# mfkiwl/coxgraph

Measured on AMD Instinct MI355X. Metric: 640x480 depth frames/sec fused (TSDF, 5 cm voxels) per node; submap registrations/sec reported alongside, higher is better.
Workload: dtype f32; 1 GPU; configs[1]: 1 client per GPU, 640x480 synthetic depth stream, 5 cm voxels, merged integrator semantics (the reference's configured method is fast; bit-exact vs CPU oracle), points resident in HBM; points_per_frame=307200, method=merged, clients=1

## Files before the change

coxgraph_amd/csrc/cox_integrator.hip:

```cpp
#include <hip/hip_runtime.h>

#include <algorithm>
#include <chrono>
#include <cmath>
#include <cstring>
#include <limits>
#include <new>
#include <string>
#include <vector>

#include "../../include/coxgraph_hip_history.h"
#include "../../include/coxgraph_hip_selftest.h"
#include "cox_host.hpp"
#include "cox_plan.hpp"
#include "cox_sort.hpp"
#include "cox_threads.hpp"

using namespace cox;
using cox_plan::IntegratorPlan;
using cox_plan::LayerUpdate;

#include "cox_frame.hpp"
#include "cox_raygen.hpp"
#include "cox_walk.hpp"
#include "cox_pieces.hpp"
#include "cox_fast.hpp"
#include "cox_apply_records.hpp"
#include "cox_apply_tile.hpp"
#include "cox_frontend.hpp"

static_assert(cox_plan::kAxisCapSmall == kAxisCapSmall && cox_plan::kTileShift == kTileShift && cox_plan::kBigChunk == kBigChunk &&
                  cox_plan::kBigChunkMin == kBigChunkMin && cox_plan::kFastMaxRounds == kFastMaxRounds && cox_plan::kFastShortMax == kFastShortMax &&
                  cox_plan::kFastRelaxGroups == kFastRelaxGroups && cox_plan::kCopyGroups == kCopyGroups,
              "cox_plan.hpp decides with the kernels' own constants");

constexpr int kStatRing = 8;
constexpr int kFrameSets = 6;
constexpr int kStageSets = 3;
constexpr int kInputSets = kFrameSets;
using cox_plan::kNumStages;

struct FrameSet {
  FrameParams* d_params = nullptr;
  Counters* cnt = nullptr;
  RayArrays rays{};
  u64* fh_keys = nullptr;
  u32* fh_first = nullptr;
  hipEvent_t done = nullptr;
  hipEvent_t params_copied = nullptr;
  hipEvent_t hand[kNumStages - 1] = {};
  bool used = false;
};
struct BundleSet {
  u32 *pslot = nullptr, *skey[2] = {nullptr, nullptr}, *sval[2] = {nullptr, nullptr}, *bstart = nullptr;
  u32 *hrank = nullptr, *head = nullptr;
  SortInfo* sort_info = nullptr;
  hipEvent_t done = nullptr;
  bool used = false;
};
struct RecordSet {
  u32 *rec_key[2] = {nullptr, nullptr}, *rec_ray[2] = {nullptr, nullptr};
  u32 *piece_front = nullptr, *piece_back = nullptr, *piece_wsum = nullptr;
  uint8_t* lin8 = nullptr;
  u32 *pkey[2] = {nullptr, nullptr}, *pstart[2] = {nullptr, nullptr}, *prl[2] = {nullptr, nullptr};
  u64* pbkey = nullptr;
  u32 *plen = nullptr, *pdest = nullptr;
  u32* touched_slots = nullptr;
  u64* ft_keys = nullptr;
  u32* ft_ord = nullptr;
  int4* ord_info = nullptr;
  u32 *blk_beg = nullptr, *blk_end = nullptr;
  u32 *big_of_tile = nullptr, *big_acc = nullptr;
  u32* blk_list = nullptr;
  uint2* big_chunks = nullptr;
  u32 big_chunk_cap = 0;
  SortInfo* sort_info = nullptr;
  hipEvent_t done = nullptr;
// ... 390 lines not shown
static int points_sort_passes(const cox_integrator* I) { return (ceil_log2(next_pow2(static_cast<u64>(I->pcap) + 1)) + 1 + 10) / 11; }

static int stage_hash(const StageCtx& c, hipStream_t s) {
  cox_integrator* I = c.I;
  FrameSet& F = *c.F;
  BundleSet& B = *c.B;
  const bool by_value = (I->method == COX_METHOD_MERGED) && !I->graphs_on;
  if (!by_value) {
    COX_HIP(hipMemcpyAsync(F.d_params, &I->h_params[c.slot], sizeof(FrameParams), hipMemcpyHostToDevice, s));
    if (c.n_dev) hipLaunchKernelGGL(k_params_count, dim3(1), dim3(1), 0, s, F.d_params, c.n_dev);
  }
  COX_HIP(hipMemsetAsync(F.cnt, 0, sizeof(Counters), s));
  if (I->method == COX_METHOD_MERGED) {
    const u32 n = I->pcap;
    {
      TimedRegion t(I, COX_KC_BUNDLE_HASH, s);
      const bool self_clean = !I->cfg.enable_anti_grazing;
      if (!self_clean) COX_HIP(hipMemsetAsync(F.fh_keys, 0xFF, sizeof(u64) * I->fh_cap + sizeof(u32) * I->fh_cap, s));
      hipLaunchKernelGGL(k_bundle_insert, grid_for(n), dim3(256), 0, s, F.d_params, I->h_params[c.slot], by_value ? 1 : 0, c.n_dev, F.fh_keys, F.fh_first,
                         I->fh_cap - 1, B.pslot, F.cnt);
    }
  }
  return COX_OK;
}
static int stage_point_sort(const StageCtx& c, hipStream_t s) {
  cox_integrator* I = c.I;
  FrameSet& F = *c.F;
  BundleSet& B = *c.B;
  if (I->method == COX_METHOD_MERGED) {
    const u32 n = I->pcap;
    const SortWorkspace& ws = (I->st_alt && (c.slot & 1)) ? I->sort_pts_alt : I->sort_pts;
    const bool counted = static_cast<u64>(n) <= static_cast<u64>(kRsMaxTiles) * kRsTile;
    {
      TimedRegion t(I, COX_KC_BUNDLE_HASH, s);
      hipLaunchKernelGGL(k_bundle_keys, grid_for(n, kHeadTile), dim3(kKeysThreads), 0, s, F.d_params, F.fh_keys, F.fh_first, B.pslot, B.skey[0], B.sval[0], B.hrank, B.head,
                         B.sort_info, counted ? ws.counts : nullptr, ws.totals);
    }
    const bool self_clean = !I->cfg.enable_anti_grazing;
    const BundleBounds bounds{F.d_params, B.head, B.hrank, B.pslot, B.bstart, F.cnt, self_clean ? F.fh_keys : nullptr, F.fh_first, I->fh_cap - 1};
    TimedRegion t(I, COX_KC_POINT_SORT, s);
    (void)radix_sort_pairs<11, BundleBounds>(B.skey[0], B.sval[0], B.skey[1], B.sval[1], &F.d_params->n_points, n, n, 0, true, points_sort_passes(I), ws, B.sort_info,
                                             s, nullptr, nullptr, counted, bounds);
  }
  return COX_OK;
}
static FrameBlocks frame_blocks(const cox_integrator* I, const RecordSet& S) { return FrameBlocks{S.ft_keys, S.ft_ord, S.touched_slots, I->layer->ht_cap - 1}; }
static void record_walk(const StageCtx& c, hipStream_t s) {
  cox_integrator* I = c.I;
  const IntegratorPlan& P = I->plan;
  FrameSet& F = *c.F;
  RecordSet& S = *c.S;
  const u32 fh_mask = I->fh_cap - 1;
  const FrameBlocks FB = frame_blocks(I, S);
  if (P.small_axis_cap)
    hipLaunchKernelGGL(k_touch_wave<kAxisCapSmall>, dim3(P.grid_touch), dim3(256), 0, s, F.d_params, F.rays, FB, S.rec_key[1], I->rcap, F.cnt, F.fh_keys, fh_mask);
  else
    hipLaunchKernelGGL(k_touch_wave<kAxisCapLarge>, dim3(2048), dim3(256), 0, s, F.d_params, F.rays, FB, S.rec_key[1], I->rcap, F.cnt, F.fh_keys, fh_mask);
  hipLaunchKernelGGL(k_emit_wave, dim3(P.grid_touch), dim3(256), 0, s, F.d_params, F.rays, FB, S.rec_key[1], S.rec_key[0], S.rec_ray[0], I->rcap, F.cnt, S.sort_info,
                     F.fh_keys, fh_mask, P.emit_flags());
}
static bool binds_in_apply(const cox_integrator* I) { return I->method == COX_METHOD_MERGED && I->plan.layer_update == LayerUpdate::RecordTiles; }
static void bind_blocks(const StageCtx& c, hipStream_t s) {
  cox_integrator* I = c.I;
  if (binds_in_apply(I)) return;
  hipLaunchKernelGGL(k_bind_blocks, dim3(16), dim3(256), 0, s, layer_view(I->layer), frame_blocks(I, *c.S), c.S->ord_info, c.F->cnt, I->layer->d_err);
}
static int stage_merge(const StageCtx& c, hipStream_t s) {
  cox_integrator* I = c.I;
  FrameSet& F = *c.F;
  BundleSet& B = *c.B;
  const u32 n = I->pcap;
  if (I->method == COX_METHOD_MERGED) {
    BundleView V{{B.skey[0], B.skey[1]}, {B.sval[0], B.sval[1]}, B.sort_info};
    {
      TimedRegion t(I, COX_KC_MERGE, s);
      hipLaunchKernelGGL(k_bundle_merge, dim3(I->plan.grid_merge), dim3(256), 0, s, F.d_params, V, B.bstart, F.rays, F.cnt,
                         I->plan.walks_pieces() ? (I->plan.small_axis_cap ? kAxisCapSmall : kAxisCapLarge) : 0u);
    }
    const bool odd = I->st_alt && (c.slot & 1);
    const ScanWorkspace& ws = odd ? I->scanws_a : I->scanws_b;
    if (!I->plan.walks_pieces()) {
      hipLaunchKernelGGL(k_scan_small, dim3(1), dim3(1024), 0, s, F.rays.nsteps, F.rays.rec_off, &F.cnt->n_ray_slots, I->pcap, &F.cnt->n_records);
    } else if (I->plan.small_axis_cap) {
      hipLaunchKernelGGL(k_scan_small2, dim3(1), dim3(1024), 0, s, F.rays.nsteps, F.rays.rec_off, &F.cnt->n_records, F.rays.pbound, F.rays.piece_off,
                         &F.cnt->n_piece_slots, &F.cnt->n_ray_slots, I->pcap);
    } else {
      exclusive_scan_u32(F.rays.nsteps, F.rays.rec_off, &F.cnt->n_ray_slots, I->pcap, I->pcap, &F.cnt->n_records, ws, s);
      exclusive_scan_u32(F.rays.pbound, F.rays.piece_off, &F.cnt->n_ray_slots, I->pcap, I->pcap, &F.cnt->n_piece_slots, ws, s);
    }
  } else {
    hipLaunchKernelGGL(k_rays_simple, grid_for(n), dim3(256), 0, s, F.d_params, F.rays, F.cnt);
  }
  return COX_OK;
}
static int stage_touch(const StageCtx& c, hipStream_t s) {
  cox_integrator* I = c.I;
  const IntegratorPlan& P = I->plan;
  FrameSet& F = *c.F;
  RecordSet& S = *c.S;
  const LayerView L = layer_view(I->layer);
  const u32 fh_mask = I->fh_cap - 1;
  if (P.walk_on_raygen) {
    bind_blocks(c, s);
    return COX_OK;
  }
  TimedRegion t_walk(I, COX_KC_TOUCH_EMIT, s);
  if (P.walks_pieces()) {
    const PieceArrays PA{S.pkey[0], S.pstart[0], S.prl[0], S.pbkey};
#define COX_LAUNCH_WALK(CAP, DEFER)                                                                                                                       \
  hipLaunchKernelGGL((k_touch_pieces<CAP, DEFER>), dim3(2048), dim3(256), 0, s, F.d_params, F.rays, L, S.touched_slots, S.lin8, PA, I->rcap, I->piece_cap, \
                     F.cnt, I->layer->d_err)
    if (P.expands_pieces()) {
      if (P.small_axis_cap)
        COX_LAUNCH_WALK(kAxisCapSmall, true);
      else
        COX_LAUNCH_WALK(kAxisCapLarge, true);
      hipLaunchKernelGGL(k_piece_touch, dim3(2048), dim3(256), 0, s, F.d_params, L, PA, I->rcap, I->piece_cap, S.touched_slots, F.cnt, I->layer->d_err);
      const u32 ht_cap = I->layer->ht_cap;
      hipLaunchKernelGGL(k_ord_flags, grid_for(ht_cap, 256, 4096), dim3(256), 0, s, F.d_params, L);
      exclusive_scan_u32(L.ht_ord, L.ht_ord, nullptr, ht_cap, ht_cap, &F.cnt->n_touched, I->scanws_h, s);
      hipLaunchKernelGGL(k_ord_scatter, grid_for(ht_cap, 256, 4096), dim3(256), 0, s, F.d_params, L, S.touched_slots);
    } else if (P.small_axis_cap) {
      COX_LAUNCH_WALK(kAxisCapSmall, false);
    } else {
      COX_LAUNCH_WALK(kAxisCapLarge, false);
    }
#undef COX_LAUNCH_WALK
    hipLaunchKernelGGL(k_piece_keys, dim3(1024), dim3(256), 0, s, L, S.pkey[0], I->rcap, I->piece_cap, F.cnt, S.sort_info, S.touched_slots, S.ord_info,
                       P.expands_pieces() ? P.tile_shift - kTileShift : 0u);
    return COX_OK;
// ... 333 lines not shown
    COX_HIP(hipEventRecord(F.hand[0], I->st[0]));
    if (I->has_producer) {
      COX_HIP(hipEventRecord(I->ev_inputs_read, I->st[0]));
      COX_HIP(hipStreamWaitEvent(I->producer, I->ev_inputs_read, 0));
    }
    if (in.consumed) COX_HIP(hipEventRecord(in.consumed, I->st[0]));
    COX_HIP(hipGetLastError());
    auto back = [ctx, job, foreign_writer]() -> int {
      cox_integrator* I = ctx.I;
      FrameSet& F = *ctx.F;
      RecordSet& S = *ctx.S;
      cox_layer* Lh = I->layer;
      tl_frame_no = ctx.frame;
      COX_HIP(hipStreamWaitEvent(I->st[1], F.hand[0], 0));
      COX_TRY(fast_solve(ctx, job));
      COX_HIP(hipEventRecord(F.hand[2], I->st[1]));
      COX_HIP(hipStreamWaitEvent(I->st[3], F.hand[2], 0));
      if (foreign_writer) cox_layer_wait_writes(Lh, I->st[3]);
      COX_TRY(run_stage(3, ctx));
      COX_TRY(run_stage(4, ctx));
      COX_TRY(run_stage(5, ctx));
      COX_HIP(hipEventRecord(F.done, I->st[5]));
      COX_HIP(hipEventRecord(S.done, I->st[5]));
      COX_HIP(hipEventRecord(Lh->last_write, I->st[5]));
      Lh->has_write = true;
      F.used = true;
      S.used = true;
      COX_HIP(hipGetLastError());
      return COX_OK;
    };
    if (I->submitter && !caller_waits) {
      I->submitter->post(back);
    } else {
      if (I->submitter) I->submitter->wait_outstanding(0);
      COX_TRY(back());
    }
    I->last_has_counts = true;
    return COX_OK;
  }
  auto chain = [](const StageCtx& x, int k) -> int {
    cox_integrator* I = x.I;
    const hipStream_t sk = stage_stream(I, k, x.slot);
    if (k > 0 && sk != stage_stream(I, k - 1, x.slot)) COX_HIP(hipStreamWaitEvent(sk, x.F->hand[k - 1], 0));
    COX_TRY(run_stage(k, x));
    if (k + 1 < kNumStages && stage_stream(I, k + 1, x.slot) != sk) COX_HIP(hipEventRecord(x.F->hand[k], sk));
    return COX_OK;
  };
  const hipStream_t s_h = stage_stream(I, 0, slot), s_m = stage_stream(I, 2, slot);
  if (F.used && s_h != I->st[5]) COX_HIP(hipStreamWaitEvent(s_h, F.done, 0));
  if (B.used && (I->st_alt || s_h != s_m)) COX_HIP(hipStreamWaitEvent(s_h, B.done, 0));
  COX_TRY(chain(ctx, 0));
  COX_HIP(hipEventRecord(F.params_copied, s_h));
  COX_TRY(chain(ctx, 1));
  COX_TRY(chain(ctx, 2));
  COX_HIP(hipEventRecord(B.done, s_m));
  B.used = true;
  if (I->has_producer) {
    COX_HIP(hipEventRecord(I->ev_inputs_read, s_m));
    COX_HIP(hipStreamWaitEvent(I->producer, I->ev_inputs_read, 0));
  }
  if (in.consumed) COX_HIP(hipEventRecord(in.consumed, s_m));
  if (I->plan.walk_on_raygen) {
    if (S.used) COX_HIP(hipStreamWaitEvent(s_m, S.done, 0));
    {
      TimedRegion t_walk(I, COX_KC_TOUCH_EMIT, s_m);
      record_walk(ctx, s_m);
    }
    if (stage_stream(I, 3, slot) != s_m) COX_HIP(hipEventRecord(F.hand[2], s_m));
  }
  COX_HIP(hipGetLastError());
  auto stage_b = [ctx, chain, foreign_writer]() -> int {
    cox_integrator* I = ctx.I;
    FrameSet& F = *ctx.F;
    RecordSet& S = *ctx.S;
    cox_layer* Lh = I->layer;
    if (S.used && I->st[3] != I->st[5]) COX_HIP(hipStreamWaitEvent(I->st[3], S.done, 0));
    if (foreign_writer) cox_layer_wait_writes(Lh, I->st[3]);
    COX_TRY(chain(ctx, 3));
    COX_TRY(chain(ctx, 4));
    COX_TRY(chain(ctx, 5));
    COX_HIP(hipEventRecord(F.done, I->st[5]));
    COX_HIP(hipEventRecord(S.done, I->st[5]));
    COX_HIP(hipEventRecord(Lh->last_write, I->st[5]));
    Lh->has_write = true;
    F.used = true;
    S.used = true;
    COX_HIP(hipGetLastError());
    return COX_OK;
  };
  if (I->submitter && !caller_waits) {
    I->submitter->post(stage_b);
  } else {
    if (I->submitter) I->submitter->wait_outstanding(0);
    COX_TRY(stage_b());
  }
  I->last_has_counts = true;
  return COX_OK;
}

static int fold_counters(cox_integrator* I) {
  if (!I->last_has_counts) return COX_OK;
  Counters& c = I->h_ring[I->frame_no % kStatRing];
  COX_HIP(hipMemcpy(&c, I->fs[I->frame_no % kFrameSets].cnt, sizeof(Counters), hipMemcpyDeviceToHost));
  if (I->last_count_on_device) {
    u32 np = 0;
    COX_HIP(hipMemcpy(&np, &I->fs[I->frame_no % kFrameSets].d_params->n_points, sizeof(u32), hipMemcpyDeviceToHost));
    I->last.n_points = np;
  }
  u64 sh[5] = {0, 0, 0, 0, 0};
  u32 max_bundle = 0, max_run = 0;
  for (int s = 0; s < 64; ++s) {
    for (int k = 0; k < 5; ++k) sh[k] += c.shard[s][k];
    max_bundle = std::max(max_bundle, c.shard[s][kShMaxBundle]);
    max_run = std::max(max_run, c.shard[s][kShMaxRun]);
  }
  I->last.max_bundle_points = max_bundle;
// ... 710 lines not shown
```

coxgraph_amd/csrc/cox_plan.hpp:

```cpp
#pragma once
#include <algorithm>
#include <cmath>
#include <cstdint>
#include <cstdio>
#include <cstdlib>
#include <cstring>
#include <string>

#include "../../include/coxgraph_hip.h"

namespace cox_plan {

#define COX_PLAN_SWITCHES(X)                                                                                                                   \
  X(APPLY) X(APPLY_WAVE) X(BIG_CHUNK) X(BUCKETS) X(COPY_THREADS) X(DEBUG) X(DEPTH_CONVERT) X(FAST_CAP) X(FAST_FENCE) X(FAST_GROUPS)             \
  X(FAST_ROUNDS) X(FAST_SEQUENTIAL) X(FAST_STREAMS) X(GRAPH) X(GRID_APPLY) X(GRID_APPLY_WAVE) X(GRID_MERGE) X(GRID_TOUCH) X(H2D) X(H2D_GROUPS) \
  X(INPUT_STREAM) X(NO_GRAPH) X(PARTITION) X(QUEUES) X(RECORD_CAP) X(SPLIT_TILES) X(STREAMS) X(STREAM_MAP) X(SUBMIT_THREAD) X(TILE) X(TIMELINE) X(WALK)       \
  X(WAVE_TILE_MAX)
#define COX_PLAN_ENUM(n) k##n,
#define COX_PLAN_NAME(n) "COX_" #n,
enum Switch { COX_PLAN_SWITCHES(COX_PLAN_ENUM) kNumSwitches };
constexpr const char* kSwitchNames[kNumSwitches] = {COX_PLAN_SWITCHES(COX_PLAN_NAME)};
#undef COX_PLAN_ENUM
#undef COX_PLAN_NAME

constexpr uint32_t kAxisCapSmall = 128;
constexpr uint32_t kTileShift = 8, kBigChunk = 4096, kBigChunkMin = 1024;
constexpr int kFastMaxRounds = 8;
constexpr uint32_t kFastCap0Max = 32, kFastShortMax = 32, kFastRelaxGroups = 128;
constexpr int kCopyGroups = 8;
constexpr int kAmpleQueues = 0;
constexpr int kMaxQueueBudget = 64;
constexpr int kNumStages = 6;

enum class LayerUpdate {
  RecordsFullSort,
  RecordTiles,
  PiecesExpand,
  PiecesApply,
};

struct FastPlan {
  int streams = 3;
  int rounds = 2;
  uint32_t cap0 = 8, cap1 = 16;
  uint32_t relax_groups = kFastRelaxGroups;
  int fences = 1;
  bool force_sequential = false;
};

struct IntegratorPlan {
  LayerUpdate layer_update = LayerUpdate::RecordTiles;
  bool bucket_partition = true;
  uint32_t tile_shift = kTileShift;
  bool wave_apply = true;
  bool split_big_tiles = true;
  uint32_t big_chunk = kBigChunk, wave_tile_max = 512;
  uint32_t grid_apply = 8192, grid_apply_wave = 2048, grid_merge = 4096, grid_touch = 2048;
  uint32_t steps_max = 0;
  bool small_axis_cap = false;
  uint32_t record_cap = 0;
  int stage_stream[kNumStages] = {0, 0, 0, 1, 1, 2};
  bool alt_raygen_stream = false;
  bool input_stream = true;
  int n_streams = 0;
  bool walk_on_raygen = false;
  bool use_graphs = false;
  bool submit_thread = true;
  int copy_threads = 3;
  bool h2d_kernel = false;
  int h2d_groups = kCopyGroups;
  bool depth_convert_on_input_stream = false;
  std::string timeline;
  bool debug = false;
  FastPlan fast;

  bool walks_pieces() const { return layer_update == LayerUpdate::PiecesExpand || layer_update == LayerUpdate::PiecesApply; }
  bool tile_apply() const { return layer_update == LayerUpdate::RecordTiles || layer_update == LayerUpdate::PiecesExpand; }
  bool expands_pieces() const { return layer_update == LayerUpdate::PiecesExpand; }
  int n_stage_streams() const { return stage_stream[kNumStages - 1] + 1; }
  int emit_flags() const { return layer_update == LayerUpdate::RecordTiles ? static_cast<int>(tile_shift | (bucket_partition ? 256u : 0u)) : 0; }
  int record_sort_passes() const { return layer_update == LayerUpdate::RecordsFullSort ? 3 : bucket_partition ? 1 : 2; }
};

inline uint32_t max_steps_per_ray(const cox_tsdf_config& cfg, float voxel_size) {
  const double reach = static_cast<double>(cfg.max_ray_length_m) + static_cast<double>(cfg.default_truncation_distance);
  const double per_axis = std::floor(reach / static_cast<double>(voxel_size)) + 3.0;
  return static_cast<uint32_t>(std::min(3.0 * per_axis + 1.0, 1.0e6));
}

template <typename Lookup>
IntegratorPlan resolve_plan(int method, const cox_tsdf_config& cfg, float voxel_size, Lookup env, int hw_queues = kAmpleQueues) {
  const char* v[kNumSwitches];
  for (int k = 0; k < kNumSwitches; ++k) v[k] = env(kSwitchNames[k]);
  auto is = [&](Switch s, const char* word) { return v[s] && std::strcmp(v[s], word) == 0; };
  auto num = [&](Switch s) { return std::atoi(v[s]); };
  const bool merged = method == COX_METHOD_MERGED, fast = method == COX_METHOD_FAST;

  IntegratorPlan p;
  p.steps_max = max_steps_per_ray(cfg, voxel_size);
  p.small_axis_cap = (p.steps_max - 1) / 3 + 2 <= kAxisCapSmall;

  const bool may_walk_pieces = merged && !cfg.enable_anti_grazing;
  p.bucket_partition = v[kBUCKETS] ? num(kBUCKETS) != 0 : p.small_axis_cap;
  if (is(kAPPLY, "records")) {
    p.layer_update = LayerUpdate::RecordsFullSort;
  } else if (may_walk_pieces && is(kAPPLY, "pieces")) {
    p.layer_update = LayerUpdate::PiecesApply;
  } else if (may_walk_pieces) {
    const bool pieces = v[kPARTITION] ? is(kPARTITION, "pieces") : !p.small_axis_cap;
    p.layer_update = pieces ? LayerUpdate::PiecesExpand : LayerUpdate::RecordTiles;
    if (v[kTILE]) p.tile_shift = num(kTILE) == 9 ? 9u : 8u;
  }
  if (v[kRECORD_CAP] && !fast && !p.walks_pieces() && num(kRECORD_CAP) > 0) p.record_cap = static_cast<uint32_t>(num(kRECORD_CAP));
  if (v[kAPPLY_WAVE]) p.wave_apply = num(kAPPLY_WAVE) != 0;
  if (v[kSPLIT_TILES]) p.split_big_tiles = num(kSPLIT_TILES) != 0;
  if (v[kBIG_CHUNK]) p.big_chunk = static_cast<uint32_t>(std::max<int>(kBigChunkMin, num(kBIG_CHUNK)));
  if (v[kWAVE_TILE_MAX]) p.wave_tile_max = num(kWAVE_TILE_MAX) == 256 ? 256u : 512u;
  if (v[kGRID_APPLY]) p.grid_apply = static_cast<uint32_t>(std::max(1, num(kGRID_APPLY)));
// ... 14 lines not shown
  const bool three_p = is(kSTREAMS, "3p");
  const bool update_heavy = !chosen && merged && p.expands_pieces();
  p.alt_raygen_stream = (width == 4 || three_p) && !fast && !v[kSTREAM_MAP] && !update_heavy && !is(kSTREAMS, "4s");
  const int* map = fast ? kFast : update_heavy ? kUpdateHeavy : three_p ? kTwo : p.alt_raygen_stream ? kParity : width == 2 ? kTwo : width == 4 ? kStaged : kSix;
  int custom[kNumStages];
  if (v[kSTREAM_MAP] && !fast) {
    const char* e = v[kSTREAM_MAP];
    bool ok = std::strlen(e) == kNumStages && e[0] == '0';
    for (int k = 0; ok && k < kNumStages; ++k) {
      custom[k] = e[k] - '0';
      ok = custom[k] >= 0 && custom[k] < kNumStages && (k == 0 || custom[k] == custom[k - 1] || custom[k] == custom[k - 1] + 1);
    }
    if (ok) map = custom;
  }
  if (fast) {
    p.fast.streams = (v[kFAST_STREAMS] && num(kFAST_STREAMS) == 1) ? 1 : 3;
    if (p.fast.streams == 1) map = kOne;
  }
  p.input_stream = !(v[kINPUT_STREAM] && num(kINPUT_STREAM) == 0);

  int budget = hw_queues;
  if (v[kQUEUES]) {
    char* end = nullptr;
    const long n = std::strtol(v[kQUEUES], &end, 10);
    if (end != v[kQUEUES] && *end == '\0' && n >= 1 && n <= kMaxQueueBudget) budget = static_cast<int>(n);
  }
  p.use_graphs = v[kGRAPH] != nullptr && v[kNO_GRAPH] == nullptr;
  if (budget > 0 && !p.use_graphs) {
    const int room = std::max(1, budget - 1);
    const bool map_chosen = fast ? v[kFAST_STREAMS] != nullptr : chosen;
    auto streams = [&] { return map[kNumStages - 1] + 1 + (p.alt_raygen_stream ? 1 : 0) + (p.input_stream ? 1 : 0); };
    if (!v[kINPUT_STREAM] && streams() > room) p.input_stream = false;
    while (!map_chosen && streams() > room && map != kOne) {
      if (fast) {
        map = kOne;
        p.fast.streams = 1;
      } else if (map == kUpdateHeavy) {
        map = kParity;
      } else if (map == kParity && p.alt_raygen_stream) {
        map = kTwo;
      } else if (p.alt_raygen_stream) {
        p.alt_raygen_stream = false;
      } else {
        map = map == kParity ? kTwo : kOne;
      }
    }
  }
  std::copy(map, map + kNumStages, p.stage_stream);
  p.n_streams = p.n_stage_streams() + (p.alt_raygen_stream ? 1 : 0) + (p.input_stream ? 1 : 0);

  {
    const bool can = merged && !p.walks_pieces() && !p.use_graphs;
    const bool rule = p.alt_raygen_stream && p.stage_stream[3] == p.stage_stream[5];
    p.walk_on_raygen = can && (is(kWALK, "raygen") ? true : is(kWALK, "update") ? false : rule);
  }

  if (fast) {
    FastPlan& f = p.fast;
    if (v[kFAST_FENCE]) f.fences = num(kFAST_FENCE);
    f.rounds = p.small_axis_cap ? 2 : kFastMaxRounds;
    if (f.rounds > 2) {
      f.cap0 = ((p.steps_max - 1) / 3 > 200) ? 32u : 16u;
      f.cap1 = 32u;
    }
    if (v[kFAST_ROUNDS]) f.rounds = std::min(kFastMaxRounds, std::max(2, num(kFAST_ROUNDS)));
    if (v[kFAST_GROUPS]) f.relax_groups = static_cast<uint32_t>(std::min(256, std::max(8, num(kFAST_GROUPS))));
    f.force_sequential = v[kFAST_SEQUENTIAL] && num(kFAST_SEQUENTIAL) != 0;
    if (v[kFAST_CAP]) {
      int a = 0, b = 0;
      const int got = std::sscanf(v[kFAST_CAP], "%d,%d", &a, &b);
      if (got >= 1 && a >= 1 && a <= static_cast<int>(kFastCap0Max)) f.cap0 = static_cast<uint32_t>(a);
      f.cap1 = std::max<uint32_t>(f.cap1, f.cap0);
      if (got >= 2 && b <= static_cast<int>(kFastShortMax) && static_cast<uint32_t>(b) >= f.cap0) f.cap1 = static_cast<uint32_t>(b);
    }
  }

  p.submit_thread = !(v[kSUBMIT_THREAD] && num(kSUBMIT_THREAD) == 0);
  if (v[kCOPY_THREADS]) p.copy_threads = std::min(15, std::max(0, num(kCOPY_THREADS)));
  p.h2d_kernel = is(kH2D, "kernel");
  if (v[kH2D_GROUPS]) p.h2d_groups = std::max(1, num(kH2D_GROUPS));
  p.depth_convert_on_input_stream = is(kDEPTH_CONVERT, "input");
  if (v[kTIMELINE]) p.timeline = v[kTIMELINE];
  p.debug = v[kDEBUG] != nullptr;
  return p;
}

}
```

coxgraph_amd/csrc/cox_raygen.hpp:

```cpp
#pragma once

__global__ void __launch_bounds__(256) k_rays_simple(const FrameParams* __restrict__ Pp, RayArrays R,
                                                     Counters* cnt) {
  const FrameParams P = *Pp;
  const u32 seq = blockIdx.x * blockDim.x + threadIdx.x;
  if (seq == 0) cnt->n_ray_slots = P.n_points;
  if (seq >= P.n_points) return;
  const u32 idx = mixed_index(seq, P.n_points);
  const F3 p{P.xyz[3 * idx], P.xyz[3 * idx + 1], P.xyz[3 * idx + 2]};
  bool clearing = false;
  const bool valid = point_valid(P, p, &clearing);
  u32 nsteps = 0, flags = 0;
  if (valid) {
    const F3 pg = transform_point(P, p);
    Dda d;
    dda_setup(d, P, pg, clearing);
    if (d.range_error) atomicOr(&cnt->err, kErrRange);
    nsteps = d.nsteps;
    flags = 1u | (clearing ? 2u : 0u);
    R.px[seq] = pg.x;
    R.py[seq] = pg.y;
    R.pz[seq] = pg.z;
    R.w[seq] = voxel_weight(P, p);
    R.color[seq] = pack_rgba_wire(P.rgba, idx);
// ... 209 lines not shown
        cnt->n_rays = carry;
        cnt->n_ray_slots = carry;
        cnt->n_sorted_valid = n_valid;
      }
    }
    if (threadIdx.x == 0) {
      scratch[4] = n;
      scratch[5] = Pp->np2;
    }
    __syncthreads();
  }
  struct Fetched {
    u32 ord, slot;
  };
  __device__ __forceinline__ bool wants(u32 key, u32 val, const u32* lds) const {
    const u32 np2 = lds[2 * kHeadLdsTiles + 5];
    return key != kInvalid && (key & (np2 - 1u)) == val;
  }
  __device__ __forceinline__ Fetched fetch(u32 key, u32 val, const u32* lds) const {
    const u32 n = lds[2 * kHeadLdsTiles + 4], np2 = lds[2 * kHeadLdsTiles + 5];
    const u32 cls = key >= np2 ? 1u : 0u;
    const u32 tile = val >> kHeadTileShift;
    u32 ord;
    if (tile < kHeadLdsTiles) {
      ord = lds[cls * kHeadLdsTiles + tile];
    } else {
      ord = lds[cls * kHeadLdsTiles + kHeadLdsTiles - 1];
      for (u32 t = kHeadLdsTiles - 1; t < tile; ++t) ord += tile_heads[4 * t + cls];
    }
    ord += hrank[val];
    return Fetched{ord < n ? ord : kInvalid, fh_keys ? pslot[mixed_index(val, n)] : kInvalid};
  }
  __device__ __forceinline__ void commit(const Fetched& f, u32 pos) const {
    if (f.ord != kInvalid) bstart[f.ord] = pos;
    if (f.slot <= fh_mask) {
      fh_keys[f.slot] = kEmptyKey;
      fh_first[f.slot] = 0xFFFFFFFFu;
    }
  }
};

typedef float MergeOp __attribute__((ext_vector_type(4)));

__device__ __forceinline__ u32 piece_bound(const Dda& d, u32 axis_cap) {
  const u32 ns = d.nsteps;
  if (ns == 0) return 0;
  const u32 gen = ns + 1;
  const u32 g0 = min(d.n_axis[0] + 2, gen), g1 = min(d.n_axis[1] + 2, gen), g2 = min(d.n_axis[2] + 2, gen);
  if (d.sgn[0] == 0 || d.sgn[1] == 0 || d.sgn[2] == 0 || g0 > axis_cap || g1 > axis_cap || g2 > axis_cap || ns > 3 * axis_cap) return ns;
  const u32 b = (ns + 63) / 64 + (d.n_axis[2] + 1) + ((d.n_axis[0] + 1) / 16 + 1) + ((d.n_axis[1] + 1) / 16 + 1) + 4;
  return min(b, ns);
}

__global__ void __launch_bounds__(256) k_bundle_merge(const FrameParams* __restrict__ Pp, BundleView V, const u32* __restrict__ bstart, RayArrays R, Counters* cnt,
                                                      u32 piece_axis_cap) {
  const FrameParams P = *Pp;
  const u32 np2 = P.np2;
  const float* __restrict__ xyz = P.xyz;
  const uint8_t* __restrict__ rgba = P.rgba;
  typedef const float __attribute__((address_space(1))) * GlobalF32;
  typedef const u32 __attribute__((address_space(1))) * GlobalU32;
  const GlobalF32 gxyz = (GlobalF32)xyz;
  const GlobalU32 grgba = (GlobalU32)rgba;
  const u32 spar = uniform_u32(V.info->parity & 1u);
  const u32* __restrict__ skey = V.key[spar];
  const u32* __restrict__ sval = V.val[spar];
  __shared__ MergeOp ops[4][64][4];
  const u32 n_bundles = uniform_u32(cnt->n_rays);
  const u32 n_valid = uniform_u32(cnt->n_sorted_valid);
  const u32 tid = blockIdx.x * blockDim.x + threadIdx.x;
  const u32 nthreads = gridDim.x * blockDim.x;
  const u32 lane = lane_id();
  const u32 role = lane & 3u;
  MergeOp(*tbl)[4] = ops[threadIdx.x >> 6];
  for (u32 task = uniform_u32(tid >> 6); task < 2 * n_bundles; task += nthreads >> 6) {
    const u32 m = task >> 1;
    const bool colour_wave = (task & 1u) != 0;
    const u32 begin = uniform_u32(bstart[m]);
    const u32 next_start = uniform_u32(bstart[min(m + 1u, n_bundles - 1u)]);
    const u32 end = (m + 1 < n_bundles) ? next_start : n_valid;
    if (colour_wave && rgba == nullptr) {
      if (lane == 0) {
        R.color[m] = 0u;
        reinterpret_cast<u32*>(R.q)[static_cast<size_t>(m) * 8u + 5u] = 0u;
      }
      continue;
    }
    auto gather = [&](bool has, u32 sv, float& x, float& y, float& z, u32& c) {
      x = 0.0f;
      y = 0.0f;
      z = 0.0f;
      c = 0u;
      if (has) {
        const u32 idx = mixed_index(sv, P.n_points);
        x = gxyz[3 * idx];
        y = gxyz[3 * idx + 1];
        z = gxyz[3 * idx + 2];
        if (colour_wave) c = grgba[idx];
      }
    };
    const u32 key0 = skey[begin];
    const u32 sv_a = (begin + lane < end) ? sval[begin + lane] : 0u;
    u32 sv_b = (begin + 64u + lane < end) ? sval[begin + 64u + lane] : 0u;
    float npx, npy, npz;
    u32 ncol;
    gather(begin + lane < end, sv_a, npx, npy, npz, ncol);
    const bool clearing = uniform_u32(key0) >= np2;
    if (!colour_wave && lane == 0) atomicMax(&cnt->shard[m & 63u][kShMaxBundle], end - begin);
// ... 98 lines not shown
        if (__ballot(bad || !d_ok)) {
          val = val_in;
          nxt = tbl[0][role];
          for (u32 k = 0; k < cnt_in; ++k) {
            const MergeOp op = nxt;
            nxt = tbl[(k + 1) & 63u][role];
            val = (val * op.x + op.y) / op.z;
          }
        }
      } else {
#define COX_COLOUR_STEP(op)                                 \
  {                                                         \
    const float x = val * (op).x + (op).y;                  \
    const float t = truncf(x);                              \
    val = (x - t >= 0.5f) ? t + 1.0f : t;                   \
  }
        MergeOp a0 = tbl[0][role], a1 = tbl[1][role], a2 = tbl[2][role], a3 = tbl[3][role];
        for (u32 k = 0; k < cnt_in; k += 8) {
          const u32 kb = (k + 4) & 63u;
          const MergeOp b0 = tbl[kb][role], b1 = tbl[kb + 1][role], b2 = tbl[kb + 2][role], b3 = tbl[kb + 3][role];
          __builtin_amdgcn_sched_barrier(0);
          COX_COLOUR_STEP(a0)
          COX_COLOUR_STEP(a1)
          COX_COLOUR_STEP(a2)
          COX_COLOUR_STEP(a3)
          __builtin_amdgcn_sched_barrier(0);
          const u32 ka = (k + 8) & 63u;
          a0 = tbl[ka][role];
          a1 = tbl[ka + 1][role];
          a2 = tbl[ka + 2][role];
          a3 = tbl[ka + 3][role];
          __builtin_amdgcn_sched_barrier(0);
          COX_COLOUR_STEP(b0)
          COX_COLOUR_STEP(b1)
          COX_COLOUR_STEP(b2)
          COX_COLOUR_STEP(b3)
          __builtin_amdgcn_sched_barrier(0);
        }
#undef COX_COLOUR_STEP
      }
      wave_lds_handover();
      W = readlane_f32(Wnext, cnt_in - 1);
    }
    if (colour_wave) {
      u32 mcolor = 0;
#pragma unroll
      for (u32 c = 0; c < 4; ++c) mcolor |= (static_cast<u32>(static_cast<int>(readlane_f32(val, c))) & 255u) << (8u * c);
      if (lane == 0) {
        R.color[m] = mcolor;
        reinterpret_cast<u32*>(R.q)[static_cast<size_t>(m) * 8u + 5u] = mcolor;
      }
    } else {
      const float mx = readlane_f32(val, 0), my = readlane_f32(val, 1), mz = readlane_f32(val, 2);
      if (lane == 0) {
        const F3 pg = transform_point(P, F3{mx, my, mz});
        Dda d;
        dda_setup(d, P, pg, clearing);
        if (d.range_error) atomicOr(&cnt->err, kErrRange);
        R.px[m] = pg.x;
        R.py[m] = pg.y;
        R.pz[m] = pg.z;
        R.w[m] = W;
        R.flags[m] = 1u | (clearing ? 2u : 0u);
        R.key[m] = key;
        R.nsteps[m] = d.nsteps;
        if (piece_axis_cap) R.pbound[m] = piece_bound(d, piece_axis_cap);
        {
          const F3 dv = pg - F3{P.tx, P.ty, P.tz};
          typedef float F4 __attribute__((ext_vector_type(4)));
          F4* q = reinterpret_cast<F4*>(R.q + static_cast<size_t>(m) * 8u);
          q[0] = F4{dv.x, dv.y, dv.z, sqrtf(dot3(dv, dv))};
          R.q[static_cast<size_t>(m) * 8u + 4u] = W;
        }
      }
    }
  }
}
```

coxgraph_amd/csrc/cox_walk.hpp:

```cpp
#pragma once

__device__ __forceinline__ bool grazing_skip(const FrameParams& P, const u64* fh_keys, u32 fh_mask, bool clearing, u64 own_key, int x, int y, int z) {
  if (!P.anti_grazing) return false;
  const u64 k = pack_key(x, y, z);
  if (!clearing && k == own_key) return false;
  return ht_find(fh_keys, fh_mask, k) != kInvalid;
}

__global__ void __launch_bounds__(256) k_touch(const FrameParams* __restrict__ Pp, RayArrays R, LayerView L, u32* __restrict__ touched_slots, Counters* cnt, u32* layer_err,
                                               const u64* __restrict__ fh_keys, u32 fh_mask) {
  const FrameParams P = *Pp;
  const u32 n_slots = cnt->n_ray_slots;
  for (u32 r = blockIdx.x * blockDim.x + threadIdx.x; r < n_slots; r += gridDim.x * blockDim.x) {
    const u32 ns = R.nsteps[r];
    if (ns == 0) continue;
    const bool clearing = (R.flags[r] & 2u) != 0;
    const F3 pg{R.px[r], R.py[r], R.pz[r]};
    const u64 own_key = P.anti_grazing ? R.key[r] : 0ull;
    Dda d;
    dda_setup(d, P, pg, clearing);
    u64 last_bkey = kEmptyKey;
    for (u32 s = 0; s < ns; ++s) {
      const int x = d.c[0], y = d.c[1], z = d.c[2];
      dda_step(d);
// ... 227 lines not shown
__device__ __forceinline__ void touch_frame_block(const FrameBlocks& B, u64 bkey, Counters* cnt) {
  bool fresh;
  const u32 slot = ht_insert(B.keys, B.mask, bkey, &fresh);
  if (slot == kInvalid) {
    atomicOr(&cnt->err, kErrTable);
    return;
  }
  if (fresh) {
    const u32 ord = atomicAdd(&cnt->n_touched, 1u);
    B.ord[slot] = ord;
    B.slots[ord] = slot;
  }
}
__device__ __forceinline__ u32 frame_block_ord(const FrameBlocks& B, u64 bkey) {
  const u32 slot = ht_find(B.keys, B.mask, bkey);
  return slot != kInvalid ? B.ord[slot] : kInvalid;
}
__device__ __forceinline__ void bind_touched_blocks(const LayerView& L, const FrameBlocks& B, int4* __restrict__ ord_info, Counters* cnt, u32* layer_err) {
  const u32 n_touched = cnt->n_touched;
  for (u32 ord = blockIdx.x * blockDim.x + threadIdx.x; ord < n_touched; ord += gridDim.x * blockDim.x) {
    const u32 fslot = B.slots[ord];
    const u64 bkey = B.keys[fslot];
    B.keys[fslot] = kEmptyKey;
    u32 pool = kInvalid;
    bool fresh;
    const u32 slot = ht_insert(L.ht_keys, L.ht_mask, bkey, &fresh);
    if (slot == kInvalid) {
      atomicOr(layer_err, kErrTable);
    } else if (fresh) {
      pool = atomicAdd(L.d_nblocks, 1u);
      if (pool < L.capacity) {
        L.ht_vals[slot] = pool;
        L.block_keys[pool] = bkey;
        atomicAdd(&cnt->n_new_blocks, 1u);
      } else {
        atomicSub(L.d_nblocks, 1u);
        atomicOr(layer_err, kErrPool);
        pool = kInvalid;
      }
    } else {
      pool = L.ht_vals[slot];
    }
    if (pool == kInvalid) atomicOr(&cnt->err, kErrPool);
    int bx, by, bz;
    unpack_key(bkey, &bx, &by, &bz);
    ord_info[ord] = make_int4(bx * 16, by * 16, bz * 16, static_cast<int>(pool));
  }
}
__global__ void __launch_bounds__(256) k_bind_blocks(LayerView L, FrameBlocks B, int4* __restrict__ ord_info, Counters* cnt, u32* layer_err) {
  bind_touched_blocks(L, B, ord_info, cnt, layer_err);
}

template <u32 kAxisCap>
__global__ void __launch_bounds__(256) k_touch_wave(const FrameParams* __restrict__ Pp, RayArrays R, FrameBlocks B, u32* __restrict__ path_out, u32 rec_cap, Counters* cnt,
                                                    const u64* __restrict__ fh_keys, u32 fh_mask) {
  const FrameParams P = *Pp;
  __shared__ float lds_t[4][3 * kAxisCap];
  __shared__ u32 lds_path[4][3 * kAxisCap];
  const u32 n_slots = uniform_u32(cnt->n_ray_slots);
  const bool overflow = uniform_u32(cnt->n_records) > rec_cap;
  const u32 lane = lane_id();
  const u32 wave = threadIdx.x >> 6;
  float* tl = lds_t[wave];
  u32* path = lds_path[wave];
  const u32 waves_total = (gridDim.x * blockDim.x) >> 6;
  for (u32 r = uniform_u32((blockIdx.x * blockDim.x + threadIdx.x) >> 6); r < n_slots; r += waves_total) {
    const u32 ns = uniform_u32(R.nsteps[r]);
    if (ns == 0) continue;
    const u32 flags = uniform_u32(R.flags[r]);
    const bool clearing = (flags & 2u) != 0;
    const F3 pg{readlane_f32(R.px[r], 0), readlane_f32(R.py[r], 0), readlane_f32(R.pz[r], 0)};
    const u64 own_key = P.anti_grazing ? R.key[r] : 0ull;
    Dda d;
    dda_setup(d, P, pg, clearing);
    const bool par = wave_ray_path<kAxisCap>(d, ns, tl, path, lane);
    if (lane == 0) R.flags[r] = par ? (flags & ~kRayFallback) : (flags | kRayFallback);
    if (par) {
      const u32 off = uniform_u32(R.rec_off[r]);
      u64 carry = kEmptyKey;
      for (u32 base = 0; base < ns; base += 64) {
        const u32 s = base + lane;
        const bool act = s < ns;
        u64 bkey = kEmptyKey;
        bool skip = false;
        if (act) {
          const u32 p = path[s];
          if (!overflow) path_out[off + s] = p;
          const int x = d.c[0] + static_cast<int>(p & 1023u) * d.sgn[0];
          const int y = d.c[1] + static_cast<int>((p >> 10) & 1023u) * d.sgn[1];
          const int z = d.c[2] + static_cast<int>(p >> 20) * d.sgn[2];
          skip = grazing_skip(P, fh_keys, fh_mask, clearing, own_key, x, y, z);
          bkey = pack_key(x >> 4, y >> 4, z >> 4);
        }
        const u64 kept = __ballot(act && !skip);
        const u64 kept_below = kept & ((1ull << lane) - 1ull);
        const int src = kept_below ? (63 - __clzll(static_cast<long long>(kept_below))) : 0;
        const u64 prev_kept = __shfl(bkey, src, 64);
        const u64 prev = kept_below ? prev_kept : carry;
        if (act && !skip && bkey != prev) touch_frame_block(B, bkey, cnt);
        if (kept) carry = __shfl(bkey, 63 - __clzll(static_cast<long long>(kept)), 64);
      }
      wave_lds_handover();
    } else if (lane == 0) {
      u64 last_bkey = kEmptyKey;
      for (u32 s = 0; s < ns; ++s) {
        const int x = d.c[0], y = d.c[1], z = d.c[2];
        dda_step(d);
        if (grazing_skip(P, fh_keys, fh_mask, clearing, own_key, x, y, z)) continue;
        const u64 bkey = pack_key(x >> 4, y >> 4, z >> 4);
        if (bkey == last_bkey) continue;
        last_bkey = bkey;
        touch_frame_block(B, bkey, cnt);
      }
    }
  }
}

__global__ void __launch_bounds__(256) k_emit_wave(const FrameParams* __restrict__ Pp, RayArrays R, FrameBlocks B, const u32* __restrict__ path_in, u32* __restrict__ rec_key,
                                                   u32* __restrict__ rec_ray, u32 rec_cap, Counters* cnt, SortInfo* sort_info,
                                                   const u64* __restrict__ fh_keys, u32 fh_mask, int by_block) {
  const FrameParams P = *Pp;
  const u32 n_slots = uniform_u32(cnt->n_ray_slots);
  const bool overflow = uniform_u32(cnt->n_records) > rec_cap;
  if (blockIdx.x == 0 && threadIdx.x == 0) {
    u32 bits = 12;
    while ((1ull << (bits - 12)) < static_cast<u64>(cnt->n_touched) + 1ull) ++bits;
    const u32 shift = static_cast<u32>(by_block) & 255u;
    sort_info->nbits = overflow ? 0u : ((by_block & 256) ? min(bits - shift, 12u) : bits - shift);
    sort_info->parity = 0;
    sort_info->base = shift;
    if (overflow) atomicOr(&cnt->err, kErrRecords);
  }
  if (overflow) return;
  const u32 lane = lane_id();
  const u32 waves_total = (gridDim.x * blockDim.x) >> 6;
  for (u32 r = uniform_u32((blockIdx.x * blockDim.x + threadIdx.x) >> 6); r < n_slots; r += waves_total) {
    const u32 ns = uniform_u32(R.nsteps[r]);
    if (ns == 0) continue;
    const u32 flags = uniform_u32(R.flags[r]);
    const bool clearing = (flags & 2u) != 0;
    const u32 off = uniform_u32(R.rec_off[r]);
    const F3 pg{readlane_f32(R.px[r], 0), readlane_f32(R.py[r], 0), readlane_f32(R.pz[r], 0)};
    const u64 own_key = P.anti_grazing ? R.key[r] : 0ull;
    Dda d;
    dda_setup(d, P, pg, clearing);
    if (!(flags & kRayFallback)) {
      u64 carry_key = kEmptyKey;
      u32 carry_ord = kInvalid;
      for (u32 base = 0; base < ns; base += 64) {
        const u32 s = base + lane;
        const bool act = s < ns;
        u64 bkey = kEmptyKey;
        bool skip = false;
        u32 lin = 0;
        if (act) {
          const u32 p = path_in[off + s];
          const int x = d.c[0] + static_cast<int>(p & 1023u) * d.sgn[0];
          const int y = d.c[1] + static_cast<int>((p >> 10) & 1023u) * d.sgn[1];
          const int z = d.c[2] + static_cast<int>(p >> 20) * d.sgn[2];
          skip = grazing_skip(P, fh_keys, fh_mask, clearing, own_key, x, y, z);
          bkey = pack_key(x >> 4, y >> 4, z >> 4);
          lin = static_cast<u32>((x & 15) | ((y & 15) << 4) | ((z & 15) << 8));
        }
        u64 prev = __shfl_up(bkey, 1, 64);
        if (lane == 0) prev = carry_key;
        const bool is_head = act && bkey != prev;
        u32 ord = kInvalid;
        if (is_head) {
          ord = frame_block_ord(B, bkey);
        }
        const u64 heads = __ballot(is_head);
        const u64 below = heads & ((lane == 63) ? ~0ull : ((2ull << lane) - 1ull));
        const int src = below ? (63 - __clzll(static_cast<long long>(below))) : 0;
        const u32 head_ord = static_cast<u32>(__shfl(static_cast<int>(ord), src, 64));
        const u32 my_ord = below ? head_ord : carry_ord;
        if (act) {
          rec_key[off + s] = (skip || my_ord == kInvalid) ? kInvalid : ((my_ord << 12) | lin);
          rec_ray[off + s] = r;
        }
        carry_key = __shfl(bkey, 63, 64);
        carry_ord = static_cast<u32>(__shfl(static_cast<int>(my_ord), 63, 64));
      }
    } else if (lane == 0) {
      u64 last_bkey = kEmptyKey;
      u32 last_ord = kInvalid;
      for (u32 s = 0; s < ns; ++s) {
        const int x = d.c[0], y = d.c[1], z = d.c[2];
        dda_step(d);
        u32 vid = kInvalid;
        if (!grazing_skip(P, fh_keys, fh_mask, clearing, own_key, x, y, z)) {
          const u64 bkey = pack_key(x >> 4, y >> 4, z >> 4);
          if (bkey != last_bkey) {
            last_bkey = bkey;
            last_ord = frame_block_ord(B, bkey);
          }
          if (last_ord != kInvalid) vid = (last_ord << 12) | static_cast<u32>((x & 15) | ((y & 15) << 4) | ((z & 15) << 8));
        }
        rec_key[off + s] = vid;
        rec_ray[off + s] = r;
      }
    }
  }
}
```

Baseline: 8341 frames/s.

## Fuse block-touch ray walk into bundle merge kernel

Adds a touch_in_merge plan mode in which k_bundle_merge walks each merged ray's voxel path right after DDA setup. It marks the touched frame blocks and stores the path at a fixed per-ray stride, so the separate k_touch_wave launch and its reload of ray data are skipped. k_emit_wave then reads paths by ray index times stride instead of the scanned record offset. The cost is that the merge kernel now waits on the record set's previous use. All 64 lanes take the DDA branch and reuse operand LDS as scratch, which lengthens merge and can exhaust record capacity for long rays, which then take the fallback path.

```diff
diff --git a/coxgraph_amd/csrc/cox_integrator.hip b/coxgraph_amd/csrc/cox_integrator.hip
--- a/coxgraph_amd/csrc/cox_integrator.hip
+++ b/coxgraph_amd/csrc/cox_integrator.hip
@@ -21,8 +21,8 @@
 using cox_plan::LayerUpdate;
 
 #include "cox_frame.hpp"
+#include "cox_walk.hpp"
 #include "cox_raygen.hpp"
-#include "cox_walk.hpp"
 #include "cox_pieces.hpp"
 #include "cox_fast.hpp"
 #include "cox_apply_records.hpp"
@@ -519,12 +519,14 @@
   RecordSet& S = *c.S;
   const u32 fh_mask = I->fh_cap - 1;
   const FrameBlocks FB = frame_blocks(I, S);
-  if (P.small_axis_cap)
-    hipLaunchKernelGGL(k_touch_wave<kAxisCapSmall>, dim3(P.grid_touch), dim3(256), 0, s, F.d_params, F.rays, FB, S.rec_key[1], I->rcap, F.cnt, F.fh_keys, fh_mask);
-  else
-    hipLaunchKernelGGL(k_touch_wave<kAxisCapLarge>, dim3(2048), dim3(256), 0, s, F.d_params, F.rays, FB, S.rec_key[1], I->rcap, F.cnt, F.fh_keys, fh_mask);
+  if (!P.touch_in_merge) {
+    if (P.small_axis_cap)
+      hipLaunchKernelGGL(k_touch_wave<kAxisCapSmall>, dim3(P.grid_touch), dim3(256), 0, s, F.d_params, F.rays, FB, S.rec_key[1], I->rcap, F.cnt, F.fh_keys, fh_mask);
+    else
+      hipLaunchKernelGGL(k_touch_wave<kAxisCapLarge>, dim3(2048), dim3(256), 0, s, F.d_params, F.rays, FB, S.rec_key[1], I->rcap, F.cnt, F.fh_keys, fh_mask);
+  }
   hipLaunchKernelGGL(k_emit_wave, dim3(P.grid_touch), dim3(256), 0, s, F.d_params, F.rays, FB, S.rec_key[1], S.rec_key[0], S.rec_ray[0], I->rcap, F.cnt, S.sort_info,
-                     F.fh_keys, fh_mask, P.emit_flags());
+                     F.fh_keys, fh_mask, P.emit_flags(), P.touch_in_merge ? P.steps_max : 0u);
 }
 static bool binds_in_apply(const cox_integrator* I) { return I->method == COX_METHOD_MERGED && I->plan.layer_update == LayerUpdate::RecordTiles; }
 static void bind_blocks(const StageCtx& c, hipStream_t s) {
@@ -541,8 +543,14 @@
     BundleView V{{B.skey[0], B.skey[1]}, {B.sval[0], B.sval[1]}, B.sort_info};
     {
       TimedRegion t(I, COX_KC_MERGE, s);
-      hipLaunchKernelGGL(k_bundle_merge, dim3(I->plan.grid_merge), dim3(256), 0, s, F.d_params, V, B.bstart, F.rays, F.cnt,
-                         I->plan.walks_pieces() ? (I->plan.small_axis_cap ? kAxisCapSmall : kAxisCapLarge) : 0u);
+      const u32 piece_axis_cap = I->plan.walks_pieces() ? (I->plan.small_axis_cap ? kAxisCapSmall : kAxisCapLarge) : 0u;
+      if (I->plan.touch_in_merge) {
+        RecordSet& S = *c.S;
+        const MergeTouch T{frame_blocks(I, S), S.rec_key[1], I->rcap, I->plan.steps_max, F.fh_keys, I->fh_cap - 1};
+        hipLaunchKernelGGL(k_bundle_merge<true>, dim3(I->plan.grid_merge), dim3(256), 0, s, F.d_params, V, B.bstart, F.rays, F.cnt, piece_axis_cap, T);
+      } else {
+        hipLaunchKernelGGL(k_bundle_merge<false>, dim3(I->plan.grid_merge), dim3(256), 0, s, F.d_params, V, B.bstart, F.rays, F.cnt, piece_axis_cap, MergeTouch{});
+      }
     }
     const bool odd = I->st_alt && (c.slot & 1);
     const ScanWorkspace& ws = odd ? I->scanws_a : I->scanws_b;
@@ -982,6 +990,7 @@
   COX_TRY(chain(ctx, 0));
   COX_HIP(hipEventRecord(F.params_copied, s_h));
   COX_TRY(chain(ctx, 1));
+  if (I->plan.touch_in_merge && S.used) COX_HIP(hipStreamWaitEvent(s_m, S.done, 0));
   COX_TRY(chain(ctx, 2));
   COX_HIP(hipEventRecord(B.done, s_m));
   B.used = true;
@@ -991,7 +1000,7 @@
   }
   if (in.consumed) COX_HIP(hipEventRecord(in.consumed, s_m));
   if (I->plan.walk_on_raygen) {
-    if (S.used) COX_HIP(hipStreamWaitEvent(s_m, S.done, 0));
+    if (S.used && !I->plan.touch_in_merge) COX_HIP(hipStreamWaitEvent(s_m, S.done, 0));
     {
       TimedRegion t_walk(I, COX_KC_TOUCH_EMIT, s_m);
       record_walk(ctx, s_m);
diff --git a/coxgraph_amd/csrc/cox_plan.hpp b/coxgraph_amd/csrc/cox_plan.hpp
--- a/coxgraph_amd/csrc/cox_plan.hpp
+++ b/coxgraph_amd/csrc/cox_plan.hpp
@@ -64,6 +64,7 @@
   bool input_stream = true;
   int n_streams = 0;
   bool walk_on_raygen = false;
+  bool touch_in_merge = false;
   bool use_graphs = false;
   bool submit_thread = true;
   int copy_threads = 3;
@@ -184,7 +185,8 @@
   {
     const bool can = merged && !p.walks_pieces() && !p.use_graphs;
     const bool rule = p.alt_raygen_stream && p.stage_stream[3] == p.stage_stream[5];
-    p.walk_on_raygen = can && (is(kWALK, "raygen") ? true : is(kWALK, "update") ? false : rule);
+    p.walk_on_raygen = can && ((is(kWALK, "raygen") || is(kWALK, "merge")) ? true : is(kWALK, "update") ? false : rule);
+    p.touch_in_merge = p.walk_on_raygen && p.small_axis_cap && !is(kWALK, "raygen");
   }
 
   if (fast) {
diff --git a/coxgraph_amd/csrc/cox_raygen.hpp b/coxgraph_amd/csrc/cox_raygen.hpp
--- a/coxgraph_amd/csrc/cox_raygen.hpp
+++ b/coxgraph_amd/csrc/cox_raygen.hpp
@@ -285,8 +285,16 @@
   return min(b, ns);
 }
 
+struct MergeTouch {
+  FrameBlocks B;
+  u32* path_out;
+  u32 rec_cap, path_stride;
+  const u64* fh_keys;
+  u32 fh_mask;
+};
+template <bool kTouch>
 __global__ void __launch_bounds__(256) k_bundle_merge(const FrameParams* __restrict__ Pp, BundleView V, const u32* __restrict__ bstart, RayArrays R, Counters* cnt,
-                                                      u32 piece_axis_cap) {
+                                                      u32 piece_axis_cap, MergeTouch T) {
   const FrameParams P = *Pp;
   const u32 np2 = P.np2;
   const float* __restrict__ xyz = P.xyz;
@@ -491,27 +499,43 @@
       }
     } else {
       const float mx = readlane_f32(val, 0), my = readlane_f32(val, 1), mz = readlane_f32(val, 2);
-      if (lane == 0) {
+      if (kTouch || lane == 0) {
         const F3 pg = transform_point(P, F3{mx, my, mz});
         Dda d;
         dda_setup(d, P, pg, clearing);
-        if (d.range_error) atomicOr(&cnt->err, kErrRange);
-        R.px[m] = pg.x;
-        R.py[m] = pg.y;
-        R.pz[m] = pg.z;
-        R.w[m] = W;
-        R.flags[m] = 1u | (clearing ? 2u : 0u);
-        R.key[m] = key;
-        R.nsteps[m] = d.nsteps;
-        if (piece_axis_cap) R.pbound[m] = piece_bound(d, piece_axis_cap);
-        {
-          const F3 dv = pg - F3{P.tx, P.ty, P.tz};
-          typedef float F4 __attribute__((ext_vector_type(4)));
-          F4* q = reinterpret_cast<F4*>(R.q + static_cast<size_t>(m) * 8u);
-          q[0] = F4{dv.x, dv.y, dv.z, sqrtf(dot3(dv, dv))};
-          R.q[static_cast<size_t>(m) * 8u + 4u] = W;
-        }
-      }
-    }
-  }
-}
+        if (lane == 0) {
+          if (d.range_error) atomicOr(&cnt->err, kErrRange);
+          R.px[m] = pg.x;
+          R.py[m] = pg.y;
+          R.pz[m] = pg.z;
+          R.w[m] = W;
+          R.flags[m] = 1u | (clearing ? 2u : 0u);
+          R.key[m] = key;
+          R.nsteps[m] = d.nsteps;
+          if (piece_axis_cap) R.pbound[m] = piece_bound(d, piece_axis_cap);
+          {
+            const F3 dv = pg - F3{P.tx, P.ty, P.tz};
+            typedef float F4 __attribute__((ext_vector_type(4)));
+            F4* q = reinterpret_cast<F4*>(R.q + static_cast<size_t>(m) * 8u);
+            q[0] = F4{dv.x, dv.y, dv.z, sqrtf(dot3(dv, dv))};
+            R.q[static_cast<size_t>(m) * 8u + 4u] = W;
+          }
+        }
+        if constexpr (kTouch) {
+          static_assert(3 * kAxisCapSmall * (sizeof(float) + sizeof(u32)) <= sizeof(ops[0]), "the walk's scratch lies in the operand rows");
+          const u32 ns = uniform_u32(d.nsteps);
+          if (ns != 0) {
+            float* tl = reinterpret_cast<float*>(tbl);
+            u32* path = reinterpret_cast<u32*>(tbl) + 3 * kAxisCapSmall;
+            const u64 slot0 = static_cast<u64>(m) * T.path_stride;
+            const bool fits = slot0 + ns <= static_cast<u64>(T.rec_cap);
+            const bool par = touch_ray_wave<kAxisCapSmall>(P, T.B, d, ns, clearing, P.anti_grazing ? key : 0ull, tl, path, fits ? T.path_out + slot0 : nullptr, cnt,
+                                                           T.fh_keys, T.fh_mask, lane);
+            if (lane == 0 && !(par && fits)) R.flags[m] = 1u | (clearing ? 2u : 0u) | kRayFallback;
+            wave_lds_handover();
+          }
+        }
+      }
+    }
+  }
+}
diff --git a/coxgraph_amd/csrc/cox_walk.hpp b/coxgraph_amd/csrc/cox_walk.hpp
--- a/coxgraph_amd/csrc/cox_walk.hpp
+++ b/coxgraph_amd/csrc/cox_walk.hpp
@@ -303,6 +303,50 @@
 }
 
 template <u32 kAxisCap>
+__device__ __forceinline__ bool touch_ray_wave(const FrameParams& P, const FrameBlocks& B, Dda& d, u32 ns, bool clearing, u64 own_key, float* tl, u32* path, u32* path_dst,
+                                               Counters* cnt, const u64* __restrict__ fh_keys, u32 fh_mask, u32 lane) {
+  const bool par = wave_ray_path<kAxisCap>(d, ns, tl, path, lane);
+  if (par) {
+    u64 carry = kEmptyKey;
+    for (u32 base = 0; base < ns; base += 64) {
+      const u32 s = base + lane;
+      const bool act = s < ns;
+      u64 bkey = kEmptyKey;
+      bool skip = false;
+      if (act) {
+        const u32 p = path[s];
+        if (path_dst) path_dst[s] = p;
+        const int x = d.c[0] + static_cast<int>(p & 1023u) * d.sgn[0];
+        const int y = d.c[1] + static_cast<int>((p >> 10) & 1023u) * d.sgn[1];
+        const int z = d.c[2] + static_cast<int>(p >> 20) * d.sgn[2];
+        skip = grazing_skip(P, fh_keys, fh_mask, clearing, own_key, x, y, z);
+        bkey = pack_key(x >> 4, y >> 4, z >> 4);
+      }
+      const u64 kept = __ballot(act && !skip);
+      const u64 kept_below = kept & ((1ull << lane) - 1ull);
+      const int src = kept_below ? (63 - __clzll(static_cast<long long>(kept_below))) : 0;
+      const u64 prev_kept = __shfl(bkey, src, 64);
+      const u64 prev = kept_below ? prev_kept : carry;
+      if (act && !skip && bkey != prev) touch_frame_block(B, bkey, cnt);
+      if (kept) carry = __shfl(bkey, 63 - __clzll(static_cast<long long>(kept)), 64);
+    }
+    wave_lds_handover();
+  } else if (lane == 0) {
+    u64 last_bkey = kEmptyKey;
+    for (u32 s = 0; s < ns; ++s) {
+      const int x = d.c[0], y = d.c[1], z = d.c[2];
+      dda_step(d);
+      if (grazing_skip(P, fh_keys, fh_mask, clearing, own_key, x, y, z)) continue;
+      const u64 bkey = pack_key(x >> 4, y >> 4, z >> 4);
+      if (bkey == last_bkey) continue;
+      last_bkey = bkey;
+      touch_frame_block(B, bkey, cnt);
+    }
+  }
+  return par;
+}
+
+template <u32 kAxisCap>
 __global__ void __launch_bounds__(256) k_touch_wave(const FrameParams* __restrict__ Pp, RayArrays R, FrameBlocks B, u32* __restrict__ path_out, u32 rec_cap, Counters* cnt,
                                                     const u64* __restrict__ fh_keys, u32 fh_mask) {
   const FrameParams P = *Pp;
@@ -322,54 +366,17 @@
     const bool clearing = (flags & 2u) != 0;
     const F3 pg{readlane_f32(R.px[r], 0), readlane_f32(R.py[r], 0), readlane_f32(R.pz[r], 0)};
     const u64 own_key = P.anti_grazing ? R.key[r] : 0ull;
+    const u32 off = uniform_u32(R.rec_off[r]);
     Dda d;
     dda_setup(d, P, pg, clearing);
-    const bool par = wave_ray_path<kAxisCap>(d, ns, tl, path, lane);
+    const bool par = touch_ray_wave<kAxisCap>(P, B, d, ns, clearing, own_key, tl, path, overflow ? nullptr : path_out + off, cnt, fh_keys, fh_mask, lane);
     if (lane == 0) R.flags[r] = par ? (flags & ~kRayFallback) : (flags | kRayFallback);
-    if (par) {
-      const u32 off = uniform_u32(R.rec_off[r]);
-      u64 carry = kEmptyKey;
-      for (u32 base = 0; base < ns; base += 64) {
-        const u32 s = base + lane;
-        const bool act = s < ns;
-        u64 bkey = kEmptyKey;
-        bool skip = false;
-        if (act) {
-          const u32 p = path[s];
-          if (!overflow) path_out[off + s] = p;
-          const int x = d.c[0] + static_cast<int>(p & 1023u) * d.sgn[0];
-          const int y = d.c[1] + static_cast<int>((p >> 10) & 1023u) * d.sgn[1];
-          const int z = d.c[2] + static_cast<int>(p >> 20) * d.sgn[2];
-          skip = grazing_skip(P, fh_keys, fh_mask, clearing, own_key, x, y, z);
-          bkey = pack_key(x >> 4, y >> 4, z >> 4);
-        }
-        const u64 kept = __ballot(act && !skip);
-        const u64 kept_below = kept & ((1ull << lane) - 1ull);
-        const int src = kept_below ? (63 - __clzll(static_cast<long long>(kept_below))) : 0;
-        const u64 prev_kept = __shfl(bkey, src, 64);
-        const u64 prev = kept_below ? prev_kept : carry;
-        if (act && !skip && bkey != prev) touch_frame_block(B, bkey, cnt);
-        if (kept) carry = __shfl(bkey, 63 - __clzll(static_cast<long long>(kept)), 64);
-      }
-      wave_lds_handover();
-    } else if (lane == 0) {
-      u64 last_bkey = kEmptyKey;
-      for (u32 s = 0; s < ns; ++s) {
-        const int x = d.c[0], y = d.c[1], z = d.c[2];
-        dda_step(d);
-        if (grazing_skip(P, fh_keys, fh_mask, clearing, own_key, x, y, z)) continue;
-        const u64 bkey = pack_key(x >> 4, y >> 4, z >> 4);
-        if (bkey == last_bkey) continue;
-        last_bkey = bkey;
-        touch_frame_block(B, bkey, cnt);
-      }
-    }
   }
 }
 
 __global__ void __launch_bounds__(256) k_emit_wave(const FrameParams* __restrict__ Pp, RayArrays R, FrameBlocks B, const u32* __restrict__ path_in, u32* __restrict__ rec_key,
                                                    u32* __restrict__ rec_ray, u32 rec_cap, Counters* cnt, SortInfo* sort_info,
-                                                   const u64* __restrict__ fh_keys, u32 fh_mask, int by_block) {
+                                                   const u64* __restrict__ fh_keys, u32 fh_mask, int by_block, u32 path_stride) {
   const FrameParams P = *Pp;
   const u32 n_slots = uniform_u32(cnt->n_ray_slots);
   const bool overflow = uniform_u32(cnt->n_records) > rec_cap;
@@ -396,6 +403,7 @@
     Dda d;
     dda_setup(d, P, pg, clearing);
     if (!(flags & kRayFallback)) {
+      const u32* __restrict__ path_ray = path_in + (path_stride ? static_cast<u64>(r) * path_stride : static_cast<u64>(off));
       u64 carry_key = kEmptyKey;
       u32 carry_ord = kInvalid;
       for (u32 base = 0; base < ns; base += 64) {
@@ -405,7 +413,7 @@
         bool skip = false;
         u32 lin = 0;
         if (act) {
-          const u32 p = path_in[off + s];
+          const u32 p = path_ray[s];
           const int x = d.c[0] + static_cast<int>(p & 1023u) * d.sgn[0];
           const int y = d.c[1] + static_cast<int>((p >> 10) & 1023u) * d.sgn[1];
           const int z = d.c[2] + static_cast<int>(p >> 20) * d.sgn[2];
```

After: 7963 frames/s. 0.955x the previous value.
